# hanmekim/SceneLib2

Measured on NVIDIA H100. Metric: EKF-SLAM frames/sec @320x240 N=100 feats, higher is better.
Workload: dtype f64 (EKF, scores) + u8/int32 (correlation sums)

## Files before the change

scenelib2_b200/csrc/search.cu:

```cuda
#include "sl2_context.cuh"
#include "sl2_ptx.cuh"
#include "sl2_score.cuh"

using namespace sl2;

namespace {

__device__ __forceinline__ void tma_load_3d(uint32_t dst, const CUtensorMap *map, uint32_t bar,
                                            int c0, int c1, int c2) {
  asm volatile(
      "cp.async.bulk.tensor.3d.shared::cluster.global.mbarrier::complete_tx::bytes "
      "[%0], [%1, {%3, %4, %5}], [%2];" ::"r"(dst),
      "l"(map), "r"(bar), "r"(c0), "r"(c1), "r"(c2)
      : "memory");
}

struct SearchLayout {
  int tcw, tch;
  int list, bar, vtab, per_warp;
};
__host__ __device__ inline SearchLayout search_layout(int tile_w, int tile_h, int box) {
  SearchLayout l;
  l.tcw = tile_w - 15 - box + 1;
  l.tch = tile_h - box + 1;
  const int tile_bytes = ((tile_w * tile_h + 16 + 127) / 128) * 128;
  const int max_tasks = l.tcw * ((l.tch + SL2_STRIP - 1) / SL2_STRIP);
  const int list_bytes = ((max_tasks * 4 + 15) / 16) * 16;
  const int col_bytes = ((l.tcw * 4 + 15) / 16) * 16;
  const int vtab_bytes = l.tch * 16 > col_bytes ? l.tch * 16 : col_bytes;
  l.list = tile_bytes;
  l.bar = tile_bytes + list_bytes;
  l.vtab = l.bar + 16;
  l.per_warp = ((l.vtab + vtab_bytes + 127) / 128) * 128;
  return l;
}

struct DumpPtrs {
  double *corr;
  double *sd;
  uint8_t *inside;
  int *box;
  int cap;
};

template <int BOX>
__device__ __forceinline__ void window_row(const uint32_t *wp, int sh, uint32_t (&sw)[(BOX + 3) / 4]) {
  constexpr int NW = (BOX + 3) / 4;
  constexpr uint32_t LASTMASK = (BOX % 4 == 0) ? 0xffffffffu : ((1u << (8 * (BOX % 4))) - 1u);
  uint32_t w[NW + 1];
#pragma unroll
  for (int k = 0; k <= NW; ++k) w[k] = wp[k];
#pragma unroll
  for (int k = 0; k < NW; ++k) sw[k] = __funnelshift_r(w[k], w[k + 1], sh);
  sw[NW - 1] &= LASTMASK;
}

template <int BOX>
__device__ __forceinline__ float approx_score(uint32_t ax, uint32_t a1, uint32_t a2, int Sg0, float V0f) {
  constexpr uint32_t NN = BOX * BOX, T100u = 100u * NN * NN;
  const uint32_t V1u = NN * a2 - a1 * a1;
  if (V1u > T100u) {
    float num;
    if constexpr (BOX <= 11) {
      num = (float)((int)NN * (int)ax - Sg0 * (int)a1);
    } else {
      num = (float)((long long)NN * (long long)ax - (long long)Sg0 * (long long)a1);
    }
    const float rho = num * rsqrtf(V0f * (float)V1u);
    return fmaf(-2.0f, rho, 2.0f);
  }
  return V1u == T100u ? -3.0e38f : __int_as_float(0x7f800000);
}

__host__ __device__ constexpr int filter_strip(int box) { return box <= 11 ? 8 : 16; }

template <int BOX, bool FILTER, bool JOBS = false>
__global__ void __launch_bounds__(SL2_SEARCH_WARPS * 32, FILTER ? (BOX <= 11 ? 4 : 3) : 2)
    search_kernel(const __grid_constant__ CUtensorMap tmap, const Sl2Dev d, const SearchLaunch L,
                  const DumpPtrs dump) {
  constexpr int NW = (BOX + 3) / 4;
  constexpr int HALF = (BOX - 1) / 2;
  constexpr int V = FILTER ? filter_strip(BOX) : SL2_STRIP;
  extern __shared__ __align__(128) uint8_t smem[];
  pdl_prologue();

  const int warp = threadIdx.x >> 5, lane = threadIdx.x & 31;
  const int groups = (L.jobs_per_stream + SL2_SEARCH_WARPS - 1) / SL2_SEARCH_WARPS;
  const int sl = blockIdx.x / groups;
  const int r = (blockIdx.x % groups) * SL2_SEARCH_WARPS + warp;
  if (r >= L.jobs_per_stream) return;
  const int job = sl * L.jobs_per_stream + r;
  const int feat = L.job_feat[job];
  const double P00 = L.job_puinv[job * 3 + 0], P01 = L.job_puinv[job * 3 + 1],
               P11 = L.job_puinv[job * 3 + 2];
  const double cx = L.job_centre[job * 2 + 0], cy = L.job_centre[job * 2 + 1];
  if (feat < 0) return;
  const int s = L.stream_lo + sl;

  const int TW = d.tile_w, TH = d.tile_h;
  const SearchLayout lay = search_layout(TW, TH, BOX);
  const int TCW = lay.tcw, TCH = lay.tch;
  uint8_t *tile = smem + (size_t)warp * lay.per_warp;
  uint32_t *list = reinterpret_cast<uint32_t *>(tile + lay.list);
  const uint32_t bar = smem_u32(tile + lay.bar);
  double2 *vtab = reinterpret_cast<double2 *>(tile + lay.vtab);
  short2 *colrange = reinterpret_cast<short2 *>(vtab);
  const uint32_t tile_s = smem_u32(tile);

  if (lane == 0) {
    mbar_init(bar, 1);
    fence_barrier_init();
    fence_proxy_async();
  }
  __syncwarp();

  const int uc = __double2int_rz(add_(cx, 0.5));
  const int vc = __double2int_rz(add_(cy, 0.5));
  const SearchBox sb = search_box(P00, P01, P11, uc, vc, stream_width(d.cams[s]), stream_height(d.cams[s]), HALF);
  const Ellipse ell = make_ellipse(P00, P01, P11);
  const int CW = sb.cols(), CH = sb.rows();
  const int x0 = uc + sb.us - HALF, y0 = vc + sb.vs - HALF;
  if (!FILTER && lane == 0) {
    dump.box[0] = sb.us; dump.box[1] = sb.uf; dump.box[2] = sb.vs; dump.box[3] = sb.vf;
    dump.box[4] = uc; dump.box[5] = vc;
  }

  const int img = L.slot * d.B + s;
  const auto stage = [&](int tx0, int ty0) {
    if (lane == 0) {
      mbar_expect_tx(bar, (uint32_t)(TW * TH));
      tma_load_3d(tile_s, &tmap, bar, (x0 + tx0) & ~15, y0 + ty0, img);
    }
  };
  if (CW > 0 && CH > 0) stage(0, 0);

  uint32_t T[BOX][NW];
  {
    const uint32_t *pp = reinterpret_cast<const uint32_t *>(
        JOBS ? L.job_patches + (size_t)job * (BOX * 16) : d.patches + ((size_t)s * d.Nmax + feat) * (BOX * 16));
#pragma unroll
    for (int rr = 0; rr < BOX; ++rr)
#pragma unroll
      for (int k = 0; k < NW; ++k) T[rr][k] = __ldg(pp + rr * 4 + k);
  }
  int Sg0 = 0, Sg0sq = 0;
#pragma unroll
  for (int rr = 0; rr < BOX; ++rr)
#pragma unroll
    for (int k = 0; k < NW; ++k) {
      Sg0 = __dp4a(T[rr][k], 0x01010101u, (uint32_t)Sg0);
      Sg0sq = __dp4a(T[rr][k], T[rr][k], (uint32_t)Sg0sq);
    }
  const PatchConst pconst = patch_const(BOX, Sg0, Sg0sq);
  const double V0d = fma(pconst.n, (double)Sg0sq, -((double)Sg0 * (double)Sg0));
  const float V0f = (float)V0d;
  const bool patch_ok = !(pconst.sigmag0 < 10.0);
  float bmin = 3.0e38f;

  ScanBest best;
  uint32_t phase = 0;

  if (CW > 0 && CH > 0) {
    for (int ty0 = 0; ty0 < CH; ty0 += TCH) {
      for (int tx0 = 0; tx0 < CW; tx0 += TCW) {
        const int tcw = min(TCW, CW - tx0), tch = min(TCH, CH - ty0);
        const int xoff = (x0 + tx0) & 15;
        if (tx0 != 0 || ty0 != 0) stage(tx0, ty0);
        const int nstrips = (tch + V - 1) / V;
        const int ntask = tcw * nstrips;
        int nlist = 0;
        if constexpr (FILTER) {
          const int vbase = sb.vs + ty0;
          const double r2p11 = 1.0 / (2.0 * P11);
          const float r2p11f = (float)r2p11;
          for (int cu = lane; cu < tcw; cu += 32) {
            const Ellipse::Col col = ell.col((double)(sb.us + tx0 + cu));
            auto inside = [&](int cv) { return ell.inside(col, (double)(vbase + cv)); };
            int lo, hi;
            bool scan = !(P11 > 1e-7) || !(P11 < 1e7);
            if (!scan) {
              const double vx = -col.b * r2p11;
              const double disc = col.b * col.b - 4.0 * P11 * (col.a - 9.0);
              const float r = disc > 0.0 ? __fsqrt_rn((float)disc) * r2p11f : 0.0f;
              const float lo_f = fminf(fmaxf(ceilf((float)vx - r) - (float)vbase, -1.0f), (float)tch);
              const float hi_f = fminf(fmaxf(floorf((float)vx + r) - (float)vbase, -1.0f), (float)tch);
              lo = max(0, min(tch - 1, (int)lo_f));
              hi = max(0, min(tch - 1, (int)hi_f));
              if (hi < lo) hi = lo;
              int it = 0;
              while (lo > 0 && it < 16 && inside(lo - 1)) { --lo; ++it; }
              while (lo <= hi && it < 16 && !inside(lo)) { ++lo; ++it; }
              if (it >= 16) {
                scan = true;
              } else if (lo > hi) {
                const int v0 = max(0, min(tch - 1, __float2int_rn((float)vx) - vbase));
                const int c0 = max(0, v0 - 1), c1 = min(tch - 1, v0 + 1);
                for (int cv = c0; cv <= c1; ++cv)
                  if (inside(cv)) scan = true;
              } else {
                while (hi < tch - 1 && it < 16 && inside(hi + 1)) { ++hi; ++it; }
                while (hi > lo && it < 16 && !inside(hi)) { --hi; ++it; }
                if (it >= 16) scan = true;
              }
            }
            if (scan) {
              lo = tch;
              hi = -1;
              for (int cv = 0; cv < tch; ++cv)
                if (inside(cv)) {
                  lo = min(lo, cv);
                  hi = cv;
                }
            }
            colrange[cu] = make_short2((short)lo, (short)hi);
          }
          __syncwarp();
          for (int sk = 0; sk < nstrips; ++sk) {
            const int st = (sk & 1) ? (nstrips - 1) / 2 + (sk + 1) / 2 : (nstrips - 1) / 2 - sk / 2;
            for (int cu0 = 0; cu0 < tcw; cu0 += 32) {
              const int cu = cu0 + lane;
              uint32_t entry = 0;
              if (cu < tcw) {
                const short2 rg = colrange[cu];
                const int jlo = max((int)rg.x - st * V, 0), jhi = min(min((int)rg.y - st * V, V - 1), tch - 1 - st * V);
                if (jlo <= jhi) {
                  const uint32_t mask = ((1u << (jhi + 1)) - 1u) & ~((1u << jlo) - 1u);
                  entry = (uint32_t)cu | ((uint32_t)st << 8) | (mask << 16);
                }
              }
              const uint32_t bal = __ballot_sync(0xffffffffu, entry != 0);
              if (entry) list[nlist + __popc(bal & ((1u << lane) - 1u))] = entry;
              nlist += __popc(bal);
            }
          }
        } else {
        for (int cv = lane; cv < tch; cv += 32) {
          const double dv = (double)(sb.vs + ty0 + cv);
          vtab[cv] = make_double2(dv, ell.vterm(dv));
        }
        __syncwarp();
        for (int t0 = 0; t0 < ntask; t0 += 32) {
          const int t = t0 + lane;
          uint32_t entry = 0;
          if (t < ntask) {
            const int sk = t / tcw, cu = t - sk * tcw;
            const int st = (sk & 1) ? (nstrips - 1) / 2 + (sk + 1) / 2 : (nstrips - 1) / 2 - sk / 2;
            const Ellipse::Col col = ell.col((double)(sb.us + tx0 + cu));
            uint32_t mask = 0;
#pragma unroll
            for (int j = 0; j < V; ++j) {
              const int cv = st * V + j;
              if (cv < tch) {
                const double2 tv = vtab[cv];
                mask |= (ell.inside(col, tv.x, tv.y) ? 1u : 0x100u) << j;
              }
            }
            if (mask) entry = (uint32_t)cu | ((uint32_t)st << 8) | (mask << 16);
          }
          const uint32_t bal = __ballot_sync(0xffffffffu, entry != 0);
          if (entry) list[nlist + __popc(bal & ((1u << lane) - 1u))] = entry;
          nlist += __popc(bal);
        }
        }
        __syncwarp();
        mbar_wait(bar, phase);
        phase ^= 1;

        const int tw4 = TW >> 2;
        if constexpr (FILTER) {
          static_assert(V <= 16, "the task entry holds a 16-bit candidate mask");
          static_assert(V >= SL2_STRIP, "the task list is sized for strips of SL2_STRIP candidates");
          for (int l0 = 0; l0 < nlist; l0 += 32) {
            float cap[V];
#pragma unroll
            for (int j = 0; j < V; ++j) cap[j] = __int_as_float(0x7f800000);
            int cv0 = 0, cand0 = 0;
            int sh = 0;
            const uint32_t *wbase = nullptr;
            if (l0 + lane < nlist && patch_ok) {
              const uint32_t e = list[l0 + lane];
              const int cu = e & 0xff, st = (e >> 8) & 0xff;
              const uint32_t m_in = e >> 16;
              cv0 = st * V;
              cand0 = (tx0 + cu) * CH + (ty0 + cv0);
              const int cx = cu + xoff;
              sh = (cx & 3) * 8;
              wbase = reinterpret_cast<const uint32_t *>(tile) + (cx >> 2);
              uint32_t ax[V], h1[V], h2[V], s1 = 0, s2 = 0;
              float lmin = bmin;
#pragma unroll
              for (int j = 0; j < V; ++j) ax[j] = 0;
#pragma unroll
              for (int rr = 0; rr < V + BOX - 1; ++rr) {
                uint32_t sw[NW];
                window_row<BOX>(wbase + min(cv0 + rr, TH - 1) * tw4, sh, sw);
                if (rr < V) {
                  h1[rr] = s1;
                  h2[rr] = s2;
                }
#pragma unroll
                for (int k = 0; k < NW; ++k) {
                  s1 = __dp4a(sw[k], 0x01010101u, s1);
                  s2 = __dp4a(sw[k], sw[k], s2);
                }
#pragma unroll
                for (int j = 0; j < V; ++j) {
                  const int t = rr - j;
                  if (t >= 0 && t < BOX) {
#pragma unroll
                    for (int k = 0; k < NW; ++k) ax[j] = __dp4a(sw[k], T[t][k], ax[j]);
                  }
                }
                const int j = rr - (BOX - 1);
                if (j >= 0 && ((m_in >> j) & 1u)) {
                  cap[j] = approx_score<BOX>(ax[j], s1 - h1[j], s2 - h2[j], Sg0, V0f);
                  if (cap[j] > -1.0e38f) lmin = fminf(lmin, cap[j]);
                }
              }
              bmin = lmin;
            }
#pragma unroll
            for (int o = 16; o > 0; o >>= 1) bmin = fminf(bmin, __shfl_xor_sync(0xffffffffu, bmin, o));
            const float thr = bmin + 1.0e-5f;
            uint32_t surv = 0;
#pragma unroll
            for (int j = 0; j < V; ++j) surv |= (cap[j] <= thr ? 1u : 0u) << j;
            while (surv) {
              const int j = __ffs(surv) - 1;
              surv &= surv - 1;
              uint32_t ax = 0, a1 = 0, a2 = 0;
#pragma unroll
              for (int t = 0; t < BOX; ++t) {
                uint32_t sw[NW];
                window_row<BOX>(wbase + (cv0 + j + t) * tw4, sh, sw);
#pragma unroll
                for (int k = 0; k < NW; ++k) {
                  ax = __dp4a(sw[k], T[t][k], ax);
                  a1 = __dp4a(sw[k], 0x01010101u, a1);
                  a2 = __dp4a(sw[k], sw[k], a2);
                }
              }
              double sg1;
              const double corr = exact_score_fn(pconst, (double)(int)a1, (double)(int)a2, (double)(int)ax, &sg1);
              if (!(sg1 < 10.0)) best.offer(corr, cand0 + j);
            }
          }
        } else {
          for (int l0 = 0; l0 < nlist; l0 += 32) {
            if (l0 + lane >= nlist) continue;
            uint32_t ax[V], a1[V], a2[V];
#pragma unroll
            for (int j = 0; j < V; ++j) ax[j] = a1[j] = a2[j] = 0;
            const uint32_t e = list[l0 + lane];
            const int cu = e & 0xff, st = (e >> 8) & 0xff;
            const uint32_t m_in = (e >> 16) & 0xff, m_all = m_in | ((e >> 24) & 0xff);
            const int cv0 = st * V;
            const int cx = cu + xoff;
            const int sh = (cx & 3) * 8;
            const uint32_t *wbase = reinterpret_cast<const uint32_t *>(tile) + (cx >> 2);
#pragma unroll
            for (int rr = 0; rr < V + BOX - 1; ++rr) {
              uint32_t sw[NW];
              window_row<BOX>(wbase + min(cv0 + rr, TH - 1) * tw4, sh, sw);
              uint32_t rs = 0, rq = 0;
#pragma unroll
              for (int k = 0; k < NW; ++k) {
                rs = __dp4a(sw[k], 0x01010101u, rs);
                rq = __dp4a(sw[k], sw[k], rq);
              }
#pragma unroll
              for (int j = 0; j < V; ++j) {
                const int t = rr - j;
                if (t >= 0 && t < BOX) {
#pragma unroll
                  for (int k = 0; k < NW; ++k) ax[j] = __dp4a(sw[k], T[t][k], ax[j]);
                  a1[j] += rs;
                  a2[j] += rq;
                }
              }
            }
#pragma unroll
            for (int j = 0; j < V; ++j) {
              if ((m_all >> j) & 1u) {
                const double Sg1d = (double)(int)a1[j], Sg1sqd = (double)(int)a2[j],
                             Sg0g1d = (double)(int)ax[j];
                double sigmag1;
                const double corr = exact_score_fn(pconst, Sg1d, Sg1sqd, Sg0g1d, &sigmag1);
                const int ui = tx0 + cu, vi = ty0 + cv0 + j;
                const int idx = ui * CH + vi;
                const bool inside = (m_in >> j) & 1u;
                if (idx < dump.cap) {
                  dump.corr[idx] = corr;
                  dump.sd[idx] = sigmag1;
                  dump.inside[idx] = inside ? 1 : 0;
                }
                if (inside && patch_ok && !(sigmag1 < 10.0)) best.offer(corr, idx);
              }
            }
          }
        }
        __syncwarp();
        fence_proxy_async();
      }
    }
  }

  best.warp_reduce();
  if (lane == 0) {
    const int2 uv = best.idx >= 0 ? scan_position(best.idx, CH, uc + sb.us, vc + sb.vs) : make_int2(-1, -1);
    const int u = uv.x, v = uv.y;
    const uint8_t ok = best.found();
    if (L.out_uv) {
      L.out_uv[job * 2 + 0] = u;
      L.out_uv[job * 2 + 1] = v;
    }
    if (L.out_found) L.out_found[job] = ok;
    if (L.out_best) L.out_best[job] = best.corr;
    if (L.scatter_to_features) {
      const size_t f = (size_t)s * d.Nmax + feat;
      d.z_uv[f * 2 + 0] = u;
      d.z_uv[f * 2 + 1] = v;
      d.found[f] = ok;
      d.best[f] = best.corr;
    }
  }
}

size_t search_smem_bytes(const Sl2Dev &d) {
  return (size_t)SL2_SEARCH_WARPS * search_layout(d.tile_w, d.tile_h, d.box).per_warp;
}

template <bool FILTER>
cudaError_t launch(const Sl2Dev &d, const CUtensorMap &tmap, const SearchLaunch &L, const DumpPtrs &dump,
                   Sl2Queue q) {
  return sl2_with_box(d.box, [&](auto box) {
    const int groups = (L.jobs_per_stream + SL2_SEARCH_WARPS - 1) / SL2_SEARCH_WARPS;
    const int grid = groups * L.stream_cnt;
    if (grid <= 0) return cudaSuccess;
    constexpr int BOX = decltype(box)::value;
    auto kern = search_kernel<BOX, FILTER>;
    if constexpr (FILTER)
      if (L.job_patches) kern = search_kernel<BOX, true, true>;
    return sl2_launch_kernel(kern, dim3(grid), dim3(SL2_SEARCH_WARPS * 32), search_smem_bytes(d), q,
                             sl2_use_pdl(L.stream_cnt), tmap, d, L, dump);
  });
}

}

cudaError_t sl2_configure_search(const Sl2Dev &d) {
  const int smem = (int)search_smem_bytes(d);
  return sl2_with_box(d.box, [&](auto box) {
    constexpr int BOX = decltype(box)::value;
    cudaError_t e = cudaFuncSetAttribute(search_kernel<BOX, true>, cudaFuncAttributeMaxDynamicSharedMemorySize, smem);
    if (e == cudaSuccess)
      e = cudaFuncSetAttribute(search_kernel<BOX, true, true>, cudaFuncAttributeMaxDynamicSharedMemorySize, smem);
    if (e == cudaSuccess)
      e = cudaFuncSetAttribute(search_kernel<BOX, false>, cudaFuncAttributeMaxDynamicSharedMemorySize, smem);
    return e;
  });
}

cudaError_t sl2_launch_search(const Sl2Dev &d, const CUtensorMap &tmap, const SearchLaunch &L, Sl2Queue q) {
  return launch<true>(d, tmap, L, DumpPtrs{}, q);
}

static cudaError_t sl2_launch_score_map(const Sl2Dev &d, const CUtensorMap &tmap, int stream_id, int slot,
                                        const double *centre_dev, const double *puinv_dev, const int *feat_dev,
                                        int *box_dev, double *corr_dev, double *sd_dev, uint8_t *inside_dev, int cap,
                                        Sl2Queue q) {
  SearchLaunch L = {};
  L.job_centre = centre_dev;
  L.job_puinv = puinv_dev;
  L.job_feat = feat_dev;
  L.jobs_per_stream = 1;
  L.stream_lo = stream_id;
  L.stream_cnt = 1;
  L.slot = slot;
  const DumpPtrs dump = {corr_dev, sd_dev, inside_dev, box_dev, cap};
  return launch<false>(d, tmap, L, dump, q);
}

extern "C" {

int sl2_patch_search(sl2_ctx *c, int32_t s, int32_t slot, int32_t n, const int32_t *feat_index,
                     const double *centre, const double *PuInv3, int32_t *u, int32_t *v,
                     uint8_t *found, double *best) {
  if (n > 0 && !feat_index) return fail(c, SL2_ERR_ARG, "sl2_patch_search: feat_index is null");
  if (bad_stream(c, s) || bad_slot(c, slot) || n < 0 || !centre || !PuInv3)
    return fail(c, SL2_ERR_ARG, "patch search: bad argument");
  if (n == 0) return SL2_OK;
  int rc = check_feature_indices(c, s, feat_index, n, "patch search: feature index out of range");
  if (rc) return rc;
  const size_t N = n;
  Stage ce{STAGE_IN, 16 * N, centre}, pu{STAGE_IN, 24 * N, PuInv3}, fe{STAGE_IN, 4 * N, feat_index},
      uv{STAGE_OUT, 8 * N}, fd{STAGE_OUT, N}, be{STAGE_OUT, 8 * N};
  rc = staged_call(c, {&ce, &pu, &fe, &uv, &fd, &be}, [] {}, [&] {
    SearchLaunch L = {};
    L.job_centre = ce.dev<double>();
    L.job_puinv = pu.dev<double>();
    L.job_feat = fe.dev<int>();
    L.jobs_per_stream = n;
    L.stream_lo = s;
    L.stream_cnt = 1;
    L.slot = slot;
    L.out_uv = uv.dev<int>();
    L.out_found = fd.d;
    L.out_best = be.dev<double>();
    L.scatter_to_features = 0;
    CU_TRY(c, sl2_launch_search(c->d, c->tmap, L, queue(c)));
    return SL2_OK;
  });
  if (rc) return rc;
  for (int i = 0; i < n; ++i) {
    if (u) u[i] = uv.host<int>()[2 * i];
    if (v) v[i] = uv.host<int>()[2 * i + 1];
    if (found) found[i] = fd.h[i];
    if (best) best[i] = be.host<double>()[i];
  }
  return SL2_OK;
}

int sl2_score_map(sl2_ctx *c, int32_t s, int32_t slot, int32_t feat, const double *centre,
                  const double *PuInv3, int32_t *box6, double *corr, double *sd_image,
                  uint8_t *inside, size_t cap) {
  if (bad_stream(c, s) || bad_slot(c, slot) || !centre || !PuInv3 || !box6)
    return fail(c, SL2_ERR_ARG, "sl2_score_map: bad argument");
  int rc = check_feature_indices(c, s, &feat, 1, "sl2_score_map: bad feature index");
  if (rc) return rc;
  Stage ce{STAGE_IN, 16, centre}, pu{STAGE_IN, 24, PuInv3}, fe{STAGE_IN, 4, &feat}, bx{STAGE_OUT, 24},
      co{STAGE_OUT, 8 * cap}, sd{STAGE_OUT, 8 * cap}, in{STAGE_OUT, cap};
  rc = staged_call(c, {&ce, &pu, &fe, &bx, &co, &sd, &in}, [] {}, [&] {
    CU_TRY(c, cudaMemsetAsync(bx.d, 0xff, in.d + cap - bx.d, c->stream));
    CU_TRY(c, sl2_launch_score_map(c->d, c->tmap, s, slot, ce.dev<double>(), pu.dev<double>(), fe.dev<int>(),
                                   bx.dev<int>(), co.dev<double>(), sd.dev<double>(), in.d, (int)cap, queue(c)));
    return SL2_OK;
  });
  if (rc) return rc;
  memcpy(box6, bx.h, 24);
  if (corr) memcpy(corr, co.h, 8 * cap);
  if (sd_image) memcpy(sd_image, sd.h, 8 * cap);
  if (inside) memcpy(inside, in.h, cap);
  return SL2_OK;
}

}
```

scenelib2_b200/csrc/sl2_score.cuh:

```cuda
#pragma once
#include "sl2_common.cuh"

namespace {

constexpr double CORRMAX = 1000000.0;
constexpr double CORRTHRESH = 0.40;

struct PatchConst {
  double n, sigmag0, A0, g0s, Sg0x2;
};

__device__ __noinline__ double exact_score_fn(const PatchConst pc, double Sg1d, double Sg1sqd,
                                              double Sg0g1d, double *sigma1_out) {
  const double g1bar = div_(Sg1d, pc.n);
  const double varg1 = sub_(div_(Sg1sqd, pc.n), mul_(g1bar, g1bar));
  const double sigmag1 = sqrt_(varg1);
  *sigma1_out = sigmag1;
  if (pc.sigmag0 == 0.0) return (sigmag1 == 0.0) ? 0.0 : 1.0;
  if (sigmag1 == 0.0) return 1.0;
  const double k = sub_(pc.g0s, div_(g1bar, sigmag1));
  double C = add_(pc.A0, div_(Sg1sqd, varg1));
  C = add_(C, mul_(pc.n, mul_(k, k)));
  C = sub_(C, div_(mul_(Sg0g1d, 2.0), mul_(pc.sigmag0, sigmag1)));
  C = sub_(C, div_(mul_(pc.Sg0x2, k), pc.sigmag0));
  C = add_(C, div_(mul_(mul_(Sg1d, 2.0), k), sigmag1));
  return div_(C, pc.n);
}

__device__ __forceinline__ PatchConst patch_const(int box, int Sg0, int Sg0sq) {
  const double n = (double)(box * box);
  const double Sg0d = (double)Sg0, Sg0sqd = (double)Sg0sq;
  const double g0bar = div_(Sg0d, n);
  const double varg0 = sub_(div_(Sg0sqd, n), mul_(g0bar, g0bar));
  const double sigmag0 = sqrt_(varg0);
  PatchConst pc;
  pc.n = n;
  pc.sigmag0 = sigmag0;
  pc.A0 = div_(Sg0sqd, varg0);
  pc.g0s = div_(g0bar, sigmag0);
  pc.Sg0x2 = mul_(Sg0d, 2.0);
  return pc;
}

struct SearchBox {
  int us, uf, vs, vf;
  __device__ __forceinline__ int cols() const { return uf - us + 1; }
  __device__ __forceinline__ int rows() const { return vf - vs + 1; }
};
__device__ __forceinline__ SearchBox search_box(double P00, double P01, double P11, int uc, int vc, int W, int H,
                                                int half) {
  const int halfwidth = __double2int_rz(div_(3.0, sqrt_(sub_(P00, div_(mul_(P01, P01), P11)))));
  const int halfheight = __double2int_rz(div_(3.0, sqrt_(sub_(P11, div_(mul_(P01, P01), P00)))));
  const int box = 2 * half + 1;
  SearchBox b = {-halfwidth, halfwidth, -halfheight, halfheight};
  if (uc + b.us - half < 0) b.us = half - uc;
  if (uc + b.uf - half > W - box) b.uf = W - box - uc + half;
  if (vc + b.vs - half < 0) b.vs = half - vc;
  if (vc + b.vf - half > H - box) b.vf = H - box - vc + half;
  return b;
}

struct Ellipse {
  double P00, b2, P11;
  struct Col {
    double a, b;
  };
  __device__ __forceinline__ Col col(double u) const { return {mul_(mul_(P00, u), u), mul_(b2, u)}; }
  __device__ __forceinline__ double vterm(double v) const { return mul_(mul_(P11, v), v); }
  __device__ __forceinline__ bool inside(Col c, double v, double vt) const {
    return add_(add_(c.a, mul_(c.b, v)), vt) < 9.0;
  }
  __device__ __forceinline__ bool inside(Col c, double v) const { return inside(c, v, vterm(v)); }
  __device__ __forceinline__ bool inside(int u, int v) const { return inside(col((double)u), (double)v); }
};
__device__ __forceinline__ Ellipse make_ellipse(double P00, double P01, double P11) {
  return {P00, mul_(2.0, P01), P11};
}

struct ScanBest {
  double corr = CORRMAX;
  int idx = -1;
  __device__ __forceinline__ void consider(double c, int i) {
    if (c < corr || (c == corr && i > idx)) {
      corr = c;
      idx = i;
    }
  }
  __device__ __forceinline__ void offer(double c, int i) {
    if (c <= CORRMAX) consider(c, i);
  }
  __device__ __forceinline__ void warp_reduce() {
#pragma unroll
    for (int o = 16; o > 0; o >>= 1) {
      const double oc = __shfl_xor_sync(0xffffffffu, corr, o);
      const int oi = __shfl_xor_sync(0xffffffffu, idx, o);
      consider(oc, oi);
    }
  }
  __device__ __forceinline__ uint8_t found() const { return (corr > CORRTHRESH) ? 0 : 1; }
};
__device__ __forceinline__ int2 scan_position(int idx, int rows, int u0, int v0) {
  return make_int2(u0 + idx / rows, v0 + idx % rows);
}

}
```

Measured before the change: 233,700.

## Split warp-uniform f64 divides across lane pairs and simplify ellipse column bounds

Warp-uniform double-precision divide/sqrt pairs in the patch constants and search-box half-widths are now computed once per lane pair, with even lanes doing one and odd lanes the other, and combined via shuffles. This halves the serial f64 divide chain each lane executes. The per-column ellipse bound search replaces iterative stepping loops with a fixed two-point check that falls back to a full scan when not settled. The strip/column list build becomes a single flattened loop over all tasks instead of nested loops. This adds shuffles, and the new bound check may fall back to a full scan more often.

After: 240,300 (median of 6 runs). 1.03x the previous value.

```diff
diff --git a/scenelib2_b200/csrc/search.cu b/scenelib2_b200/csrc/search.cu
--- a/scenelib2_b200/csrc/search.cu
+++ b/scenelib2_b200/csrc/search.cu
@@ -116,7 +116,8 @@
 
   const int uc = __double2int_rz(add_(cx, 0.5));
   const int vc = __double2int_rz(add_(cy, 0.5));
-  const SearchBox sb = search_box(P00, P01, P11, uc, vc, stream_width(d.cams[s]), stream_height(d.cams[s]), HALF);
+  const SearchBox sb =
+      search_box_warp(P00, P01, P11, uc, vc, stream_width(d.cams[s]), stream_height(d.cams[s]), HALF);
   const Ellipse ell = make_ellipse(P00, P01, P11);
   const int CW = sb.cols(), CH = sb.rows();
   const int x0 = uc + sb.us - HALF, y0 = vc + sb.vs - HALF;
@@ -151,7 +152,7 @@
       Sg0 = __dp4a(T[rr][k], 0x01010101u, (uint32_t)Sg0);
       Sg0sq = __dp4a(T[rr][k], T[rr][k], (uint32_t)Sg0sq);
     }
-  const PatchConst pconst = patch_const(BOX, Sg0, Sg0sq);
+  const PatchConst pconst = patch_const_warp(BOX, Sg0, Sg0sq);
   const double V0d = fma(pconst.n, (double)Sg0sq, -((double)Sg0 * (double)Sg0));
   const float V0f = (float)V0d;
   const bool patch_ok = !(pconst.sigmag0 < 10.0);
@@ -173,34 +174,37 @@
           const int vbase = sb.vs + ty0;
           const double r2p11 = 1.0 / (2.0 * P11);
           const float r2p11f = (float)r2p11;
+          const bool degenerate = !(P11 > 1e-7) || !(P11 < 1e7);
+          const float last = (float)(tch - 1);
           for (int cu = lane; cu < tcw; cu += 32) {
             const Ellipse::Col col = ell.col((double)(sb.us + tx0 + cu));
             auto inside = [&](int cv) { return ell.inside(col, (double)(vbase + cv)); };
-            int lo, hi;
-            bool scan = !(P11 > 1e-7) || !(P11 < 1e7);
+            auto inside_t = [&](int cv) { return inside(max(0, min(tch - 1, cv))) && cv >= 0 && cv < tch; };
+            int lo = tch, hi = -1;
+            bool scan = degenerate;
             if (!scan) {
               const double vx = -col.b * r2p11;
               const double disc = col.b * col.b - 4.0 * P11 * (col.a - 9.0);
               const float r = disc > 0.0 ? __fsqrt_rn((float)disc) * r2p11f : 0.0f;
-              const float lo_f = fminf(fmaxf(ceilf((float)vx - r) - (float)vbase, -1.0f), (float)tch);
-              const float hi_f = fminf(fmaxf(floorf((float)vx + r) - (float)vbase, -1.0f), (float)tch);
-              lo = max(0, min(tch - 1, (int)lo_f));
-              hi = max(0, min(tch - 1, (int)hi_f));
-              if (hi < lo) hi = lo;
-              int it = 0;
-              while (lo > 0 && it < 16 && inside(lo - 1)) { --lo; ++it; }
-              while (lo <= hi && it < 16 && !inside(lo)) { ++lo; ++it; }
-              if (it >= 16) {
-                scan = true;
-              } else if (lo > hi) {
+              const float tlo = (float)vx - r - (float)vbase, thi = (float)vx + r - (float)vbase;
+              const bool est_empty = !(ceilf(tlo) <= fminf(floorf(thi), last)) || !(floorf(thi) >= 0.0f);
+              bool settled = false;
+              if (!est_empty) {
+                const int L = (int)fminf(fmaxf(ceilf(tlo - 0.5f), 0.0f), last);
+                const int H = (int)fminf(fmaxf(floorf(thi + 0.5f), 0.0f), last);
+                const bool inL = inside(L), inH = inside(H);
+                const bool outL = !inside_t(inL ? L - 1 : L + 1), outH = !inside_t(inH ? H + 1 : H - 1);
+                lo = inL ? L : L + 1;
+                hi = inH ? H : H - 1;
+                settled = (inL == outL) && (inH == outH);
+              }
+              if (!settled) {
                 const int v0 = max(0, min(tch - 1, __float2int_rn((float)vx) - vbase));
                 const int c0 = max(0, v0 - 1), c1 = min(tch - 1, v0 + 1);
+                lo = tch;
+                hi = -1;
                 for (int cv = c0; cv <= c1; ++cv)
                   if (inside(cv)) scan = true;
-              } else {
-                while (hi < tch - 1 && it < 16 && inside(hi + 1)) { ++hi; ++it; }
-                while (hi > lo && it < 16 && !inside(hi)) { --hi; ++it; }
-                if (it >= 16) scan = true;
               }
             }
             if (scan) {
@@ -215,23 +219,22 @@
             colrange[cu] = make_short2((short)lo, (short)hi);
           }
           __syncwarp();
-          for (int sk = 0; sk < nstrips; ++sk) {
-            const int st = (sk & 1) ? (nstrips - 1) / 2 + (sk + 1) / 2 : (nstrips - 1) / 2 - sk / 2;
-            for (int cu0 = 0; cu0 < tcw; cu0 += 32) {
-              const int cu = cu0 + lane;
-              uint32_t entry = 0;
-              if (cu < tcw) {
-                const short2 rg = colrange[cu];
-                const int jlo = max((int)rg.x - st * V, 0), jhi = min(min((int)rg.y - st * V, V - 1), tch - 1 - st * V);
-                if (jlo <= jhi) {
-                  const uint32_t mask = ((1u << (jhi + 1)) - 1u) & ~((1u << jlo) - 1u);
-                  entry = (uint32_t)cu | ((uint32_t)st << 8) | (mask << 16);
-                }
-              }
-              const uint32_t bal = __ballot_sync(0xffffffffu, entry != 0);
-              if (entry) list[nlist + __popc(bal & ((1u << lane) - 1u))] = entry;
-              nlist += __popc(bal);
-            }
+          int sk = lane / tcw, cu = lane - sk * tcw;
+          for (int t0 = 0; t0 < ntask; t0 += 32) {
+            uint32_t entry = 0;
+            if (t0 + lane < ntask) {
+              const int st = (sk & 1) ? (nstrips - 1) / 2 + (sk + 1) / 2 : (nstrips - 1) / 2 - sk / 2;
+              const short2 rg = colrange[cu];
+              const int jlo = max((int)rg.x - st * V, 0), jhi = min(min((int)rg.y - st * V, V - 1), tch - 1 - st * V);
+              if (jlo <= jhi) {
+                const uint32_t mask = ((1u << (jhi + 1)) - 1u) & ~((1u << jlo) - 1u);
+                entry = (uint32_t)cu | ((uint32_t)st << 8) | (mask << 16);
+              }
+            }
+            const uint32_t bal = __ballot_sync(0xffffffffu, entry != 0);
+            if (entry) list[nlist + __popc(bal & ((1u << lane) - 1u))] = entry;
+            nlist += __popc(bal);
+            for (cu += 32; cu >= tcw; cu -= tcw) ++sk;
           }
         } else {
         for (int cv = lane; cv < tch; cv += 32) {
diff --git a/scenelib2_b200/csrc/sl2_score.cuh b/scenelib2_b200/csrc/sl2_score.cuh
--- a/scenelib2_b200/csrc/sl2_score.cuh
+++ b/scenelib2_b200/csrc/sl2_score.cuh
@@ -27,19 +27,41 @@
   return div_(C, pc.n);
 }
 
-__device__ __forceinline__ PatchConst patch_const(int box, int Sg0, int Sg0sq) {
+template <class Div2>
+__device__ __forceinline__ PatchConst patch_const_by(int box, int Sg0, int Sg0sq, Div2 div2) {
   const double n = (double)(box * box);
   const double Sg0d = (double)Sg0, Sg0sqd = (double)Sg0sq;
-  const double g0bar = div_(Sg0d, n);
-  const double varg0 = sub_(div_(Sg0sqd, n), mul_(g0bar, g0bar));
+  const double2 m = div2(Sg0d, n, Sg0sqd, n);
+  const double g0bar = m.x;
+  const double varg0 = sub_(m.y, mul_(g0bar, g0bar));
   const double sigmag0 = sqrt_(varg0);
+  const double2 q = div2(Sg0sqd, varg0, g0bar, sigmag0);
   PatchConst pc;
   pc.n = n;
   pc.sigmag0 = sigmag0;
-  pc.A0 = div_(Sg0sqd, varg0);
-  pc.g0s = div_(g0bar, sigmag0);
+  pc.A0 = q.x;
+  pc.g0s = q.y;
   pc.Sg0x2 = mul_(Sg0d, 2.0);
   return pc;
+}
+__device__ __forceinline__ PatchConst patch_const(int box, int Sg0, int Sg0sq) {
+  return patch_const_by(box, Sg0, Sg0sq,
+                        [](double a, double b, double c, double d) { return make_double2(div_(a, b), div_(c, d)); });
+}
+
+template <class T>
+__device__ __forceinline__ void warp_pair(T v, T &first, T &second) {
+  const int lane = threadIdx.x & 31;
+  first = __shfl_sync(0xffffffffu, v, lane & ~1);
+  second = __shfl_sync(0xffffffffu, v, lane | 1);
+}
+__device__ __forceinline__ PatchConst patch_const_warp(int box, int Sg0, int Sg0sq) {
+  return patch_const_by(box, Sg0, Sg0sq, [](double a, double b, double c, double d) {
+    const bool odd = threadIdx.x & 1;
+    double2 r;
+    warp_pair(div_(odd ? c : a, odd ? d : b), r.x, r.y);
+    return r;
+  });
 }
 
 struct SearchBox {
@@ -47,10 +69,11 @@
   __device__ __forceinline__ int cols() const { return uf - us + 1; }
   __device__ __forceinline__ int rows() const { return vf - vs + 1; }
 };
-__device__ __forceinline__ SearchBox search_box(double P00, double P01, double P11, int uc, int vc, int W, int H,
-                                                int half) {
-  const int halfwidth = __double2int_rz(div_(3.0, sqrt_(sub_(P00, div_(mul_(P01, P01), P11)))));
-  const int halfheight = __double2int_rz(div_(3.0, sqrt_(sub_(P11, div_(mul_(P01, P01), P00)))));
+__device__ __forceinline__ int search_half(double a, double P01, double b) {
+  return __double2int_rz(div_(3.0, sqrt_(sub_(a, div_(mul_(P01, P01), b)))));
+}
+__device__ __forceinline__ SearchBox clamp_search_box(int halfwidth, int halfheight, int uc, int vc, int W, int H,
+                                                      int half) {
   const int box = 2 * half + 1;
   SearchBox b = {-halfwidth, halfwidth, -halfheight, halfheight};
   if (uc + b.us - half < 0) b.us = half - uc;
@@ -58,6 +81,17 @@
   if (vc + b.vs - half < 0) b.vs = half - vc;
   if (vc + b.vf - half > H - box) b.vf = H - box - vc + half;
   return b;
+}
+__device__ __forceinline__ SearchBox search_box(double P00, double P01, double P11, int uc, int vc, int W, int H,
+                                                int half) {
+  return clamp_search_box(search_half(P00, P01, P11), search_half(P11, P01, P00), uc, vc, W, H, half);
+}
+__device__ __forceinline__ SearchBox search_box_warp(double P00, double P01, double P11, int uc, int vc, int W, int H,
+                                                     int half) {
+  const bool odd = threadIdx.x & 1;
+  int hw, hh;
+  warp_pair(search_half(odd ? P11 : P00, P01, odd ? P00 : P11), hw, hh);
+  return clamp_search_box(hw, hh, uc, vc, W, H, half);
 }
 
 struct Ellipse {
```
